# scottjones03/NoisyQuantumSimulator

Hardware: AMD Instinct MI355X
Metric: Lindblad param-points/sec (2-atom Rydberg CZ sweep); achieved HBM GB/s vs peak (higher is better)
Workload: dtype f64; 1 GPU; C2: 10k-point (Omega, Delta) LP-square CZ sweep per GPU, medium apparatus, full reference noise model (8 Lindblad channels); points_per_gpu=10000, global_points=10000, parallelism=range-shard x1, method=chebyshev (auto: 16-lane DPP-row propagator kernel, phase frame)

## Files before the change

noisyquantumsimulator_amd/csrc/ryd_engine.hip:

```cpp
#include <hip/hip_runtime.h>

#include <dlfcn.h>

#include <math.h>
#include <stdint.h>
#include <stdio.h>
#include <string.h>

#include <algorithm>
#include <atomic>
#include <chrono>
#include <complex>
#include <condition_variable>
#include <mutex>
#include <string>
#include <thread>
#include <type_traits>
#include <utility>
#include <vector>

#include "../../include/ryd_engine.h"

struct ryd_slot_work {
  void* dbuf = nullptr;
  size_t dcap = 0;
  void* hbuf = nullptr;
  size_t hcap = 0;
  hipEvent_t ev[4] = {nullptr, nullptr, nullptr, nullptr};
  bool ev_ok = false;
  hipEvent_t mark[2] = {nullptr, nullptr};
};

struct ryd_handle {
  std::vector<int> dev;
  std::vector<hipStream_t> stream;
  std::vector<ryd_slot_work> work;
  std::vector<double> timeline;
  std::mutex mu;
};

namespace {

constexpr int BLOCK = 256;
constexpr double MILLER_SEED = 1e-200;
constexpr int MILLER_MARGIN = 10;
constexpr double X_SKIP = 1e-20;
constexpr double X_CAP = 2.0e6;

struct PointP {
  double Om, Dl, V, d1;
  double gA[4], gB[4];
  double tau, xr, xi, corr, A, wmod, phoff, otau;
  int nseg;
  int64_t i, ld;
  const double* prm;
};

__device__ __forceinline__ double col(const double* p, int f, int64_t ld, int64_t i) {
  return p[(int64_t)f * ld + i];
}

template <int PROTO, typename Get>
__device__ __forceinline__ PointP load_point_with(Get get) {
  PointP q;
  q.prm = nullptr; q.ld = 0; q.i = 0;
  q.Om = get(RYD_P_OMEGA);
  q.Dl = get(RYD_P_DELTA);
  q.V = get(RYD_P_V);
  q.d1 = get(RYD_P_DELTA1);
#pragma unroll
  for (int c = 0; c < 4; ++c) {
    q.gA[c] = get(RYD_P_G1_A + c);
    q.gB[c] = get(RYD_P_G1_B + c);
  }
  q.tau = get(RYD_P_TAU);
  q.xr = q.xi = q.corr = q.A = q.wmod = q.phoff = q.otau = 0.0;
  q.nseg = 0;
  if (PROTO == RYD_PROTO_LP_SQUARE || PROTO == RYD_PROTO_LP_SHAPED) {
    q.xr = get(RYD_P_XI_RE);
    q.xi = get(RYD_P_XI_IM);
    q.corr = (PROTO == RYD_PROTO_LP_SHAPED) ? get(RYD_P_AREA_CORR) : 1.0;
  } else if (PROTO == RYD_PROTO_SMOOTH_JP) {
    q.A = get(RYD_P_A);
    q.wmod = get(RYD_P_OMEGA_MOD);
    q.phoff = get(RYD_P_PHI_OFF);
  } else {
    q.otau = get(RYD_P_OMEGA_TAU);
    q.nseg = (int)get(RYD_P_NSEG);
  }
  return q;
}

// ... 1382 lines not shown
  }
  const bool in_t = (nseg & 1) != 0;
  if (lane_ok) {
    if (in_t) rotate_coord(Rt[pl], Rs[pl], j, cp, sp);
    else rotate_coord(Rs[pl], Rt[pl], j, cp, sp);
  }
  wave_sync();
  if (!in_t && lane_ok) {
#pragma unroll
    for (int k = 0; k < 4; ++k) Rs[pl][k][j] = Rt[pl][k][j];
  }
  wave_sync();
  if (live) {
#pragma unroll
    for (int k = 0; k < 4; ++k) st[(int64_t)j * lds + 4 * i + k] = Rs[pl][k][j];
  }
  if (live && j == 0) {
    uint32_t stat = status[i];
    double pops[4], tr11 = 0.0;
    bool fin = true;
#pragma unroll
    for (int k = 0; k < 4; ++k) pops[k] = Rs[pl][k][5 * (k >> 1) + (k & 1)];
    for (int r = 0; r < NC; ++r)
      for (int k = 0; k < 4; ++k) fin = fin && isfinite(Rs[pl][k][r]);
#pragma unroll
    for (int a = 0; a < 3; ++a)
#pragma unroll
      for (int b = 0; b < 3; ++b) tr11 += Rs[pl][3][5 * a + b];
    if (!fin) stat |= RYD_STATUS_NONFINITE;
    const double nan = __builtin_nan("");
    const double avg = 0.25 * (pops[0] + pops[1] + pops[2] + pops[3]);
#pragma unroll
    for (int k = 0; k < 4; ++k) {
      sm[(int64_t)(RYD_S_POP0 + k) * ldm + i] = pops[k];
      sm[(int64_t)(RYD_S_OV_RE0 + k) * ldm + i] = nan;
      sm[(int64_t)(RYD_S_OV_IM0 + k) * ldm + i] = nan;
    }
    sm[(int64_t)RYD_S_AVG_POP * ldm + i] = avg;
    sm[(int64_t)RYD_S_CTRL_PHASE * ldm + i] = nan;
    sm[(int64_t)RYD_S_PENALTY * ldm + i] = nan;
    sm[(int64_t)RYD_S_AVG_F * ldm + i] = avg;
    sm[(int64_t)RYD_S_TRACE11 * ldm + i] = tr11;
    status[i] = stat;
  }
}

#ifndef RYD_S16_WAVES
#define RYD_S16_WAVES 4
#endif
#ifndef RYD_LP_UNSQUARED
#define RYD_LP_UNSQUARED 2
#endif
#include "ryd_sym16.inc"
#include "ryd_sched_table.inc"
#include "ryd_sched16.inc"
#include "ryd_ket_sched.inc"

constexpr int DP_BLOCK = 64;

__device__ __forceinline__ void lindblad_rhs(const Gen& A, const Gen& B, double vs,
                                             const double (&y)[25], double (&f)[25]) {
#pragma unroll
  for (int e = 0; e < 25; ++e) f[e] = 0.0;
  apply_A(A, y, f);
  apply_B(B, y, f);
  apply_V(vs, y, f);
}

struct DP {
  static constexpr double a[6][5] = {
      {0, 0, 0, 0, 0},
      {1.0 / 5, 0, 0, 0, 0},
      {3.0 / 40, 9.0 / 40, 0, 0, 0},
      {44.0 / 45, -56.0 / 15, 32.0 / 9, 0, 0},
      {19372.0 / 6561, -25360.0 / 2187, 64448.0 / 6561, -212.0 / 729, 0},
      {9017.0 / 3168, -355.0 / 33, 46732.0 / 5247, 49.0 / 176, -5103.0 / 18656}};
  static constexpr double b[6] = {35.0 / 384, 0, 500.0 / 1113, 125.0 / 192, -2187.0 / 6784, 11.0 / 84};
  static constexpr double e[6] = {71.0 / 57600, 0, -71.0 / 16695, 71.0 / 1920, -17253.0 / 339200,
                                  22.0 / 525};
  static constexpr double e7 = -1.0 / 40;
};

using KStore = double[6][25][DP_BLOCK];

template <int J>
__device__ __forceinline__ void dp_stage_input(const double (&y)[25], double hh, const KStore& ks, int lt,
                                               double (&tmp)[25]) {
#pragma unroll
  for (int e = 0; e < 25; ++e) {
    double acc = 0.0;
#pragma unroll
    for (int l = 0; l < J; ++l) acc = fma(DP::a[J][l], ks[l][e][lt], acc);
    tmp[e] = fma(hh, acc, y[e]);
  }
}

template <int PROTO>
__global__ __launch_bounds__(DP_BLOCK) void lindblad_dopri5_kernel(
    const double* __restrict__ prm, int64_t n, int64_t ldp, double* __restrict__ st, int64_t lds,
    double* __restrict__ sm, int64_t ldm, uint32_t* __restrict__ status, int n_steps, int shape,
    double rtol, double atol, int64_t max_steps) {
  __shared__ KStore ks;
  const int lt = threadIdx.x;
  const int64_t gid = (int64_t)blockIdx.x * DP_BLOCK + lt;
  const bool live = gid < 4 * n;
  const int64_t i = live ? (gid >> 2) : (n - 1);
// ... 536 lines not shown
    uint64_t keep = UINT64_MAX;
    (void)hipMemPoolSetAttribute(p, hipMemPoolAttrReleaseThreshold, &keep);
    pools[dev] = p;
  }
  return pools[dev];
}

int launch_jp_split(const ryd_batch_desc* d, const double* dp, int64_t n, int64_t ldp, double* ds,
                    int64_t lds, double* dm, int64_t ldm, uint32_t* dstat, hipStream_t stream) {
  const bool sym = (d->flags & RYD_FLAG_SYMMETRIC_ATOMS) != 0;
  int dev = 0;
  HIPCHK(hipGetDevice(&dev));
  hipMemPool_t pool = jp_pool(dev);
  if (!pool) return fail(RYD_ERR_ALLOC, "jp workspace pool creation failed");
  double* W = nullptr;
  HIPCHK(hipMallocFromPoolAsync((void**)&W, sizeof(double) * NC * NC * (size_t)n, pool, stream));
  const int ns = d->n_steps, sh = d->shape;
  int rc = launch_typed(sym ? jp_rows_kernel<true> : jp_rows_kernel<false>, (n + PPB - 1) / PPB, BLOCK, 0, stream,
                        dp, n, ldp, W, dm, ldm, dstat, ns, sh);
  if (!rc)
    rc = launch_typed(sym ? jp_frame_kernel<3, true> : jp_frame_kernel<4, false>, (n + FPB - 1) / FPB, BLOCK, 0,
                      stream, dp, n, ldp, W, ds, lds, dm, ldm, dstat, ns);
  hipError_t ef = hipFreeAsync(W, stream);
  if (rc) return rc;
  if (ef != hipSuccess) return fail(RYD_ERR_HIP, std::string("jp workspace free: ") + hipGetErrorString(ef));
  return RYD_OK;
}

template <int PROTO>
int launch_sym16(const double* dp, int64_t n, int64_t ldp, double* ds, int64_t lds, double* dm, int64_t ldm,
                 uint32_t* dstat, int ns, int sh, hipStream_t stream) {
  const int st32 = sym16_store32_enabled() && lds >= 0 && ldm >= 0 && lds <= (0x1fffffffLL - 15) / 3 &&
                   ldm <= (0x1fffffffLL - 3) / 15;
  const int bal = PROTO == RYD_PROTO_LP_SQUARE ? sym16_balance_mode() : 0;
  const int wtm = sym16_wt_mode();
  if (wtm == -2) return fail(RYD_ERR_INVALID, "RYD_S16_WT must be 0, 1 or 3");
  if (bal != 0) {
    const int cus = sym16_device_cus();
    S16Plan pl;
    const bool planned = sym16_plan(n, cus, 0, &pl);
    if (bal == 2 && !planned)
      return fail(RYD_ERR_HIP, "RYD_S16_BALANCE=2: the device's compute-unit count is not available");
    if (planned && (bal == 2 || pl.auto_on)) {
      if (const char* eg = getenv("RYD_S16_BALANCE_GPC")) {
        char* end = nullptr;
        const long over = strtol(eg, &end, 10);
        if (end == eg || *end != '\0' || over < 1 || over > S16_BAL_MAXW)
          return fail(RYD_ERR_INVALID, "RYD_S16_BALANCE_GPC must be an integer from 1 to 16");
        sym16_plan(n, cus, (int)over, &pl);
      }
      const char* eh = getenv("RYD_S16_BALANCE_NOHANDOFF");
      static_assert(RYD_P_XI_IM == 14, "the largest LP-square parameter column");
      const bool p32 = sym16_param32_enabled() && ldp <= (0x7fffffffLL / 8 - n) / 14;
      auto fb = p32 ? lindblad_sym16_kernel<RYD_PROTO_LP_SQUARE, 2> : lindblad_sym16_kernel<RYD_PROTO_LP_SQUARE, 1>;
      if (!ds)
        fb = p32 ? lindblad_sym16_nostate_kernel<RYD_PROTO_LP_SQUARE, 2>
                 : lindblad_sym16_nostate_kernel<RYD_PROTO_LP_SQUARE, 1>;
      const int noh = eh && eh[0] == '1', wt = wtm >= 0 ? wtm : S16_WT_AUTO;
      return launch_typed(fb, pl.workgroups, S16_BLOCK * pl.waves, 0, stream, dp, n, ldp, ds, lds, dm, ldm, dstat,
                          ns, pl.gpc, st32, noh, wt);
    }
  }
  if (wtm > 0) return fail(RYD_ERR_UNSUPPORTED, "RYD_S16_WT: write-through stores need the balanced launch form");
  return launch_typed(ds ? lindblad_sym16_kernel<PROTO> : lindblad_sym16_nostate_kernel<PROTO>,
                      (n + S16_PPW - 1) / S16_PPW, S16_BLOCK, 0, stream, dp, n, ldp, ds, lds, dm, ldm, dstat, ns, sh,
                      st32);
}

int launch_kernels(BatchPath path, const ryd_batch_desc* d, const double* dp, int64_t n, int64_t ldp, double* ds,
                   int64_t lds, double* dm, int64_t ldm, uint32_t* dstat, hipStream_t stream) {
  const bool sym = (d->flags & RYD_FLAG_SYMMETRIC_ATOMS) != 0, dim4 = d->dim == 4;
  const int ns = d->n_steps, sh = d->shape;
  auto go = [&](auto kernel, int64_t blocks, unsigned block, auto... more) {
    return launch_typed(kernel, blocks, block, 0, stream, dp, n, ldp, ds, lds, dm, ldm, dstat, ns, sh,
                        more...);
  };
  if (!ds && !has_twin(path)) return fail(RYD_ERR_UNSUPPORTED, "no kernel for this descriptor");
  return with_protocol(d->protocol, [&](auto proto) -> int {
    constexpr int P = decltype(proto)::value;
    constexpr bool FEW = P != RYD_PROTO_LP_SHAPED;
    KernelFn k = nullptr;
    switch (path) {
      case PATH_DOPRI5:
        return go(lindblad_dopri5_kernel<P>, (4 * n + DP_BLOCK - 1) / DP_BLOCK, DP_BLOCK, d->rtol, d->atol,
                  d->max_steps);
      case PATH_DIM4_PROP:
        if constexpr (FEW) return go(lindblad4_prop_kernel<P>, (n + D4_PPB - 1) / D4_PPB, D4_BLOCK);
        break;
      case PATH_SHAPED16:
        if constexpr (!FEW) return go(lindblad_shaped16_kernel<P>, (n + SH_PPW - 1) / SH_PPW, SH_BLOCK);
        break;
      case PATH_SYM16:
        if constexpr (FEW) return launch_sym16<P>(dp, n, ldp, ds, lds, dm, ldm, dstat, ns, sh, stream);
        break;
      case PATH_JP_SPLIT: return launch_jp_split(d, dp, n, ldp, ds, lds, dm, ldm, dstat, stream);
      case PATH_LINDBLAD_PROP:
        k = sym ? lindblad_prop_kernel<P, true> : lindblad_prop_kernel<P, false>;
        return go(k, (n + PPB - 1) / PPB, BLOCK);
      case PATH_LINDBLAD_CHEB:
        k = dim4 ? (sym ? lindblad4_cheb_kernel<P, true> : lindblad4_cheb_kernel<P, false>)
                 : (sym ? lindblad_cheb_kernel<P, true> : lindblad_cheb_kernel<P, false>);
        return go(k, (4 * n + BLOCK - 1) / BLOCK, BLOCK);
      case PATH_KET_BLOCK:
        k = ds ? (dim4 ? ket_block_kernel<P, 4> : ket_block_kernel<P, 3>)
               : (dim4 ? ket_block_nostate_kernel<P, 4> : ket_block_nostate_kernel<P, 3>);
        return go(k, (n + BLOCK - 1) / BLOCK, BLOCK);
      case PATH_KET_CHEB:
        return go(dim4 ? ket_cheb_kernel<P, 4> : ket_cheb_kernel<P, 3>, (4 * n + BLOCK - 1) / BLOCK, BLOCK);
    }
    return fail(RYD_ERR_UNSUPPORTED, "no kernel for this descriptor");
  });
}

// ... 956 lines not shown
                      int64_t ld_diag, void* stream, float* elapsed_ms) {
  return on_slot(
      h, slot, stream, elapsed_ms, [] { return RYD_OK; },
      [&](hipStream_t s) {
        return launch_derive(desc, d_in, ld_in, n, d_params, ld_params, d_warn, d_diag, ld_diag, s);
      });
}

int ryd_derive(ryd_handle* h, const ryd_derive_desc* desc, const double* in, int64_t n_cols, int64_t ld_in,
               int64_t n, double* params, int64_t ld_params, uint32_t* warn, double* diag, int64_t ld_diag) {
  if (!h || h->dev.empty() || !desc) return fail(RYD_ERR_INVALID, "derive: NULL handle/desc");
  if (n < 0 || n_cols < 0 || ld_params < n || (diag && ld_diag < n) || (n_cols > 0 && (!in || ld_in < n)))
    return fail(RYD_ERR_INVALID, "derive: bad sizes");
  for (int f = 0; f < RYD_DV_NFIELD; ++f)
    if (desc->col[f] >= n_cols) return fail(RYD_ERR_INVALID, "derive: a field's column is beyond n_cols");
  if (n == 0) return RYD_OK;
  if (!params || !warn) return fail(RYD_ERR_INVALID, "derive: NULL output");
  const int dev = h->dev[0];
  hipStream_t s = h->stream[0];
  HIPCHK(hipSetDevice(dev));
  auto al = [](size_t x) { return (x + 255) & ~(size_t)255; };
  const size_t bIn = sizeof(double) * (size_t)n_cols * n, bP = sizeof(double) * RYD_NPARAM * (size_t)n,
               bW = sizeof(uint32_t) * (size_t)n, bD = diag ? sizeof(double) * RYD_DV_NDIAG * (size_t)n : 0;
  const size_t oP = al(bIn), oW = oP + al(bP), oD = oW + al(bW), tot = oD + al(bD) + 256;
  char* buf = nullptr;
  HIPCHK(hipStreamSynchronize(s));
  HIPCHK(hipMalloc((void**)&buf, tot));
  hipError_t e = hipSuccess;
  for (int64_t c = 0; c < n_cols && e == hipSuccess; ++c)
    e = hipMemcpyAsync(buf + sizeof(double) * (size_t)c * n, in + c * ld_in, sizeof(double) * n,
                       hipMemcpyHostToDevice, s);
  if (e == hipSuccess) e = hipStreamSynchronize(s);
  int rc = RYD_OK;
  if (e == hipSuccess)
    rc = launch_derive(desc, (const double*)buf, n, n, (double*)(buf + oP), n, (uint32_t*)(buf + oW),
                       diag ? (double*)(buf + oD) : nullptr, n, s);
  if (e == hipSuccess && rc == RYD_OK) e = hipStreamSynchronize(s);
  for (int f = 0; f < RYD_NPARAM && e == hipSuccess && rc == RYD_OK; ++f)
    e = hipMemcpyAsync(params + f * ld_params, buf + oP + sizeof(double) * (size_t)f * n, sizeof(double) * n,
                       hipMemcpyDeviceToHost, s);
  if (e == hipSuccess && rc == RYD_OK) e = hipMemcpyAsync(warn, buf + oW, bW, hipMemcpyDeviceToHost, s);
  for (int k = 0; diag && k < RYD_DV_NDIAG && e == hipSuccess && rc == RYD_OK; ++k)
    e = hipMemcpyAsync(diag + k * ld_diag, buf + oD + sizeof(double) * (size_t)k * n, sizeof(double) * n,
                       hipMemcpyDeviceToHost, s);
  const hipError_t es = hipStreamSynchronize(s);
  const hipError_t ef = hipFree(buf);
  if (rc) return rc;
  if (e != hipSuccess) return fail(RYD_ERR_HIP, std::string("derive: ") + hipGetErrorString(e));
  if (ef != hipSuccess || es != hipSuccess) return fail(RYD_ERR_HIP, "derive: free/sync failed");
  return RYD_OK;
}

}
```

noisyquantumsimulator_amd/csrc/ryd_sym16.inc:

```

constexpr int S16_BLOCK = 64;
constexpr int S16_PPW = 4;

#ifndef RYD_S16_SETPRIO
#define RYD_S16_SETPRIO 1
#endif
__device__ __forceinline__ bool s16_one_round() {
  return RYD_S16_SETPRIO && gridDim.x <= 256u * 4u * (unsigned)RYD_S16_WAVES;
}
#define S16_PRIO(n) do { if (s16_one_round()) __builtin_amdgcn_s_setprio(n); } while (0)
#ifndef RYD_S16_PRIO_SPLIT
#define RYD_S16_PRIO_SPLIT 1
#endif
#ifdef RYD_S16_PROF
#define S16_MARK(k) (s16_ts[k] = (double)__builtin_readcyclecounter())
#define S16_PROF_ARG , double* s16_ts
#define S16_PROF_PASS , s16_ts
#else
#define S16_MARK(k) ((void)0)
#define S16_PROF_ARG
#define S16_PROF_PASS
#endif

#ifndef RYD_XCD_MAP
// ... 26 lines not shown
  const long long x = __builtin_bit_cast(long long, v);
  const long long y = __builtin_amdgcn_update_dpp(0LL, x, 0x150 + K, 0xF, 0xF, false);
  return __builtin_bit_cast(double, y);
}

template <typename F, int... I>
__device__ __forceinline__ void static_for_impl(F&& f, std::integer_sequence<int, I...>) {
  (f(std::integral_constant<int, I>{}), ...);
}
template <int N, typename F>
__device__ __forceinline__ void static_for(F&& f) {
  static_for_impl(f, std::make_integer_sequence<int, N>{});
}

template <int M, bool NOP>
__device__ __forceinline__ void fmac5_bcast(double& a0, double& a1, double& a2, double& a3, double& a4,
                                            double c0, double c1, double c2, double c3, double c4,
                                            double w) {
  if constexpr (NOP) asm volatile("s_nop 1" ::: "memory");
  asm volatile(
      "v_fmac_f64_dpp %0, %5, %10 row_newbcast:%11 row_mask:0xf bank_mask:0xf\n\t"
      "v_fmac_f64_dpp %1, %6, %10 row_newbcast:%11 row_mask:0xf bank_mask:0xf\n\t"
      "v_fmac_f64_dpp %2, %7, %10 row_newbcast:%11 row_mask:0xf bank_mask:0xf\n\t"
      "v_fmac_f64_dpp %3, %8, %10 row_newbcast:%11 row_mask:0xf bank_mask:0xf\n\t"
      "v_fmac_f64_dpp %4, %9, %10 row_newbcast:%11 row_mask:0xf bank_mask:0xf"
      : "+v"(a0), "+v"(a1), "+v"(a2), "+v"(a3), "+v"(a4)
      : "v"(c0), "v"(c1), "v"(c2), "v"(c3), "v"(c4), "v"(w), "i"(M));
}

template <int M0, bool NOP = true>
__device__ __forceinline__ void dot5_bcast(double& acc, double x, double o0, double o1, double o2, double o3,
                                           double o4) {
#define RYD_DOT5_BODY                                                                          \
  "v_fmac_f64_dpp %0, %1, %2 row_newbcast:%7 row_mask:0xf bank_mask:0xf\n\t"                  \
  "v_fmac_f64_dpp %0, %1, %3 row_newbcast:%8 row_mask:0xf bank_mask:0xf\n\t"                  \
  "v_fmac_f64_dpp %0, %1, %4 row_newbcast:%9 row_mask:0xf bank_mask:0xf\n\t"                  \
  "v_fmac_f64_dpp %0, %1, %5 row_newbcast:%10 row_mask:0xf bank_mask:0xf\n\t"                 \
  "v_fmac_f64_dpp %0, %1, %6 row_newbcast:%11 row_mask:0xf bank_mask:0xf"
  if constexpr (NOP) {
    asm volatile("s_nop 1\n\t" RYD_DOT5_BODY
                 : "+v"(acc)
                 : "v"(x), "v"(o0), "v"(o1), "v"(o2), "v"(o3), "v"(o4), "i"(M0), "i"(M0 + 1), "i"(M0 + 2),
                   "i"(M0 + 3), "i"(M0 + 4));
  } else {
    asm volatile(RYD_DOT5_BODY
                 : "+v"(acc)
                 : "v"(x), "v"(o0), "v"(o1), "v"(o2), "v"(o3), "v"(o4), "i"(M0), "i"(M0 + 1), "i"(M0 + 2),
                   "i"(M0 + 3), "i"(M0 + 4));
  }
#undef RYD_DOT5_BODY
}

typedef const __attribute__((address_space(3))) double lds_zero_t;
__device__ __forceinline__ void square_cols16(const double (&col)[NS], double (&acc)[NS], lds_zero_t* zl) {
  asm volatile("" ::: "memory");
#pragma unroll
  for (int k = 0; k < 5; ++k) acc[k] = 0.0;
#pragma unroll
  for (int k = 5; k < NS; ++k) {
    acc[k] = zl[k - 5];
    asm volatile("" ::: "memory");
  }
  static_for<NS>([&](auto M) {
    constexpr int m = decltype(M)::value;
    const double own = col[m];
    if constexpr (m == 0) {
      asm volatile("s_nop 1\n\tv_fmac_f64_dpp %0, %1, %2 row_newbcast:0 row_mask:0xf bank_mask:0xf"
                   : "+v"(acc[0])
                   : "v"(col[0]), "v"(own));
    } else {
      fmac5_bcast<m, m == 1>(acc[0], acc[1], acc[2], acc[3], acc[4], col[0], col[1], col[2], col[3], col[4],
                             own);
    }
    if constexpr (m >= 5) {
      fmac5_bcast<m, false>(acc[5], acc[6], acc[7], acc[8], acc[9], col[5], col[6], col[7], col[8], col[9], own);
      fmac5_bcast<m, false>(acc[10], acc[11], acc[12], acc[13], acc[14], col[10], col[11], col[12], col[13],
                            col[14], own);
    }
  });
}

__device__ __forceinline__ void fast_sincos(double x, double& s, double& c) {
  const bool ok = fabs(x) < 1e15;
  const double k = rint(x * 0.63661977236758134308);
  double r = fma(-k, 1.5707963267948966, x);
  r = fma(-k, 6.123233995736766e-17, r);
  r = fma(-k, -1.4973849048591698e-33, r);
  const double z = r * r;
  const double ps = fma(z, fma(z, fma(z, fma(z, fma(z, 1.58969099521155010221e-10, -2.50507602534068634195e-08),
                                           2.75573137070700676789e-06), -1.98412698298579493134e-04),
                               8.33333333332248946124e-03), -1.66666666666666324348e-01);
  const double sr = fma(z * r, ps, r);
  const double pc = fma(z, fma(z, fma(z, fma(z, fma(z, -1.13596475577881948265e-11, 2.08757232129817482790e-09),
                                           -2.75573143513906633035e-07), 2.48015872894767294178e-05),
                               -1.38888888888741095749e-03), 4.16666666666666019037e-02);
  const double hz = 0.5 * z, w = 1.0 - hz;
  const double cr = w + (((1.0 - w) - hz) + z * z * pc);
  const int n = (int)fma(-4.0, floor(k * 0.25), k);
  const double a = (n & 1) ? cr : sr, b = (n & 1) ? sr : cr;
  const double nan = __builtin_nan("");
  s = ok ? ((n & 2) ? -a : a) : nan;
  c = ok ? (((n + 1) & 2) ? -b : b) : nan;
}

template <int PROTO>
__device__ __forceinline__ void seg_polar(const PointP& q, int s, int n_steps, bool frame_ok, double& a,
                                          double& c, double& sn, double& dl, double& dt, bool& hold) {
  hold = false;
  dl = q.Dl;
  if (PROTO == RYD_PROTO_LP_SQUARE) {
    dt = q.tau;
    if (s == 0) {
      a = q.Om;
      c = 1.0;
      sn = 0.0;
    } else {
      a = q.Om;
      c = q.xr;
      sn = q.xi;
      if (__builtin_amdgcn_ballot_w64(!frame_ok) != 0 && !frame_ok) {
        const double m = sqrt(q.xr * q.xr + q.xi * q.xi);
        a = q.Om * m;
        c = m > 0.0 ? q.xr / m : 1.0;
        sn = m > 0.0 ? q.xi / m : 0.0;
      }
    }
  } else if (PROTO == RYD_PROTO_SMOOTH_JP) {
    a = q.Om;
    dt = q.tau / (double)n_steps;
    segment_phase<PROTO>(q, s, n_steps, c, sn);
  } else {
    const Seg g = segment<PROTO>(q, s, n_steps, RYD_SHAPE_SQUARE);
// ... 358 lines not shown
#else
  const int sq = min(sqf > keep ? sqf - keep : 0, RYD_S16_SQ_CAP);
  rep = sqf > keep ? keep : sqf;
#endif
#ifndef RYD_S16_SQ_CAP
  rep = sqf - sq;
#endif
  const double sc = act ? 2.0 / omega : 0.0;
  Gen A = make_gen(g, q.d1, q.gA, sc);
  double vs = sc * 0.5 * q.V;
  if (!act) {
    A = Gen{};
    vs = 0.0;
  }
  double v[NS];
  const int nuse0 = nuse;
  bool have = false;
  bool producer = false;
  if constexpr (SPLIT) {
    producer = ho.role == S16_BAL_PRODUCER;
    if (ho.role == S16_BAL_CONSUMER && ho.poll) have = s16_wait_flag(&ho.flag[ho.slot], ho.polls);
  }
  if (!SPLIT || !have) {
    cheb_unit16(v, r, y, act && lane_ok,
                [&](const double (&b)[NS], double (&o)[NS]) { apply_Lsym_re(A, vs, b, o); }, nuse, nexec, zl);
    if (!count) nuse = nuse0;
  }
  S16_MARK(2);
  s16_phase_prio<2>(ho);
  const int sfm = wave_max16(sqf);
  nrep = sfm > keep ? keep : sfm;
#ifndef RYD_S16_SQ_CAP
  const int smx = sfm > keep ? sfm - keep : 0;
#else
  const int smx = min(sfm > keep ? sfm - keep : 0, RYD_S16_SQ_CAP);
#endif
  int it0 = 0, it1 = smx;
  if constexpr (SPLIT) {
    const int hs = min((int)RYD_S16_BAL_HSQ, smx);
    const int l = 16 * p + r;
    if (producer) it1 = hs;
    if (have) {
      it0 = hs;
#pragma unroll
      for (int k = 0; k < NS; ++k) v[k] = ho.cols[ho.slot][k][l];
      nuse = ho.cnt[ho.slot][0][l];
      nexec = ho.cnt[ho.slot][1][l];
    }
  }
  {
    for (int it = it0; it < it1; it += 2) {
      double w[NS];
      if (RYD_S16_PRIO_SPLIT && it == ((smx >> 1) & ~1)) s16_phase_prio<1>(ho);
      if (it < sq) square_cols16(v, w, zl);
      if (it + 1 < sq) {
        square_cols16(w, v, zl);
      } else if (it < sq) {
#pragma unroll
        for (int k = 0; k < NS; ++k) v[k] = w[k];
      }
    }
  }
  if constexpr (SPLIT) {
    if (producer) {
      const int l = 16 * p + r;
#pragma unroll
      for (int k = 0; k < NS; ++k) ho.cols[ho.slot][k][l] = v[k];
      ho.cnt[ho.slot][0][l] = nuse;
      ho.cnt[ho.slot][1][l] = nexec;
#ifdef RYD_S16_PROF
      S16_MARK(3);
      ho.cnt[ho.slot][2][l] = (int)(s16_ts[3] - s16_ts[0]);
      ho.cnt[ho.slot][3][l] = (int)__builtin_amdgcn_s_getreg((4) | (0 << 6) | (31 << 11));
#endif
      __hip_atomic_store(&ho.flag[ho.slot], 1, __ATOMIC_RELEASE, __HIP_MEMORY_SCOPE_WORKGROUP);
      return true;
    }
  }
  if (count) nsq += sqf;
  S16_MARK(3);
  s16_phase_prio<1>(ho);
  wave_sync();
  if (lane_ok) {
    static_for<NS>([&](auto N) {
      constexpr int nn = decltype(N)::value;
      double w;
      if constexpr (nn == SEG_M) w = v[sym_index(3, 3)] - v[sym_index(4, 4)];
      else if constexpr (nn == SEG_Q) w = 2.0 * v[sym_index(3, 4)];
      else if constexpr (nn == SEG_P) w = v[sym_index(3, 3)] + v[sym_index(4, 4)];
      else w = v[seg_old(nn)];
      Ut[p][nn][r] = w;
    });
  }
  wave_sync();
  lds_zero_t* const src = lane_ok ? (lds_zero_t*)&Ut[p][r][0] : zl;
  double R[NS];
#pragma unroll
  for (int m = 0; m < NS; ++m) R[m] = src[m];
  static_for<NS>([&](auto N) {
    constexpr int nn = decltype(N)::value;
    if constexpr (nn == SEG_M) u[nn] = 0.5 * (R[sym_index(3, 3)] - R[sym_index(4, 4)]);
    else if constexpr (nn == SEG_Q) u[nn] = 0.5 * R[sym_index(3, 4)];
    else if constexpr (nn == SEG_P) u[nn] = 0.5 * (R[sym_index(3, 3)] + R[sym_index(4, 4)]);
    else u[nn] = R[seg_old(nn)];
  });
  S16_MARK(4);
  s16_phase_prio<0>(ho);
  return false;
}
// ... 103 lines not shown
  PointP q = load_point_with<PROTO>([&](int f) {
    const char* base = reinterpret_cast<const char*>(prm + ((int64_t)f * ldp + i0));
    asm("" : "+s"(base));
    const s16_gchar* gbase = (const s16_gchar*)base;
    return *reinterpret_cast<const s16_gdouble*>(gbase + off);
  });
  q.prm = prm;
  q.ld = ldp;
  q.i = i0 + (int64_t)(po8 >> 3);
  return q;
}

template <int PROTO>
__device__ __forceinline__ PointP load_point16_row(const double* __restrict__ prm, int64_t ldp, int64_t i0,
                                                   unsigned po8, int r) {
  static_assert(PROTO == RYD_PROTO_LP_SQUARE && RYD_P_XI_IM == NS - 1, "LP square: columns 0 .. 14, one per lane");
  const unsigned f = (unsigned)(r < NS ? r : NS - 1);
  const unsigned off = f * (8u * (unsigned)ldp) + po8;
  const char* base = reinterpret_cast<const char*>(prm + i0);
  asm("" : "+s"(base));
  const double x = *reinterpret_cast<const s16_gdouble*>((const s16_gchar*)base + off);
  double c[NS];
  static_for<NS>([&](auto K) { c[decltype(K)::value] = row_bcast<decltype(K)::value>(x); });
  PointP q = load_point_with<PROTO>([&](int k) { return c[k]; });
  q.prm = prm;
  q.ld = ldp;
  q.i = i0 + (int64_t)(po8 >> 3);
  return q;
}

__device__ __forceinline__ void s16_in_hand(PointP& q) {
  asm volatile("" : "+v"(q.Om), "+v"(q.Dl), "+v"(q.V), "+v"(q.d1), "+v"(q.gA[0]), "+v"(q.gA[1]), "+v"(q.gA[2]),
               "+v"(q.gA[3]), "+v"(q.gB[0]), "+v"(q.gB[1]), "+v"(q.gB[2]), "+v"(q.gB[3]), "+v"(q.tau), "+v"(q.xr),
               "+v"(q.xi));
}
template <int PROTO>
__device__ __forceinline__ bool point_valid_flat(const PointP& q) {
  static_assert(PROTO == RYD_PROTO_LP_SQUARE, "point_valid's LP-square predicates");
  const auto fin = [](double x) { return (int)isfinite(x); };
  int ok = (int)(q.Om > 0.0) & fin(q.Om) & fin(q.V) & fin(q.Dl) & fin(q.d1);
#pragma unroll
  for (int c = 0; c < 4; ++c)
    ok &= (int)(q.gA[c] >= 0.0) & (int)(q.gB[c] >= 0.0) & fin(q.gA[c]) & fin(q.gB[c]);
  return (ok & (int)(q.tau > 0.0) & fin(q.tau)) != 0;
}

template <int PROTO>
__global__ __launch_bounds__(S16_BLOCK) __attribute__((amdgpu_waves_per_eu(PROTO == RYD_PROTO_BANGBANG ? 3 : RYD_S16_WAVES, 8))) void
lindblad_sym16_kernel(const double* __restrict__ prm, int64_t n, int64_t ldp, double* __restrict__ st,
                      int64_t lds, double* __restrict__ sm, int64_t ldm, uint32_t* __restrict__ status,
                      int n_steps, int shape, int st32) {
  (void)shape;
  constexpr int BAL = PROTO < 0 ? 1 : 0;
  constexpr int gpc = 0, nohandoff = 0, wt = 0, p32 = 0;
  constexpr bool STATE = true;
#include "ryd_sym16_body.inc"
}

template <int PROTO>
__global__ __launch_bounds__(S16_BLOCK) __attribute__((amdgpu_waves_per_eu(PROTO == RYD_PROTO_BANGBANG ? 3 : RYD_S16_WAVES, 8))) void
lindblad_sym16_nostate_kernel(const double* __restrict__ prm, int64_t n, int64_t ldp, double* __restrict__ st,
                              int64_t lds, double* __restrict__ sm, int64_t ldm, uint32_t* __restrict__ status,
                              int n_steps, int shape, int st32) {
  (void)shape;
  constexpr int BAL = PROTO < 0 ? 1 : 0;
  constexpr int gpc = 0, nohandoff = 0, wt = 0, p32 = 0;
  constexpr bool STATE = false;
#include "ryd_sym16_body.inc"
}

template <int PROTO, int BAL>
__global__ __launch_bounds__(S16_BLOCK * S16_BAL_MAXW) __attribute__((amdgpu_waves_per_eu(RYD_S16_WAVES, 8))) void
lindblad_sym16_kernel(const double* __restrict__ prm, int64_t n, int64_t ldp, double* __restrict__ st,
                      int64_t lds, double* __restrict__ sm, int64_t ldm, uint32_t* __restrict__ status,
                      int n_steps, int gpc, int st32, int nohandoff, int wt) {
  static_assert(PROTO == RYD_PROTO_LP_SQUARE && (BAL == 1 || BAL == 2), "the balanced form is built for LP square");
  constexpr int p32 = BAL == 2;
  constexpr bool STATE = true;
#include "ryd_sym16_body.inc"
}

template <int PROTO, int BAL>
__global__ __launch_bounds__(S16_BLOCK * S16_BAL_MAXW) __attribute__((amdgpu_waves_per_eu(RYD_S16_WAVES, 8))) void
lindblad_sym16_nostate_kernel(const double* __restrict__ prm, int64_t n, int64_t ldp, double* __restrict__ st,
                              int64_t lds, double* __restrict__ sm, int64_t ldm, uint32_t* __restrict__ status,
                              int n_steps, int gpc, int st32, int nohandoff, int wt) {
  static_assert(PROTO == RYD_PROTO_LP_SQUARE && (BAL == 1 || BAL == 2), "the balanced form is built for LP square");
  constexpr int p32 = BAL == 2;
  constexpr bool STATE = false;
#include "ryd_sym16_body.inc"
}

constexpr int S16_WT_STATE = 1, S16_WT_SUMMARY = 2;
constexpr int S16_WT_AUTO = S16_WT_STATE | S16_WT_SUMMARY;
template <bool WT, typename P, typename T>
__device__ __forceinline__ void s16_store(P* ptr, T v) {
  if constexpr (WT) __hip_atomic_store(ptr, v, __ATOMIC_RELAXED, __HIP_MEMORY_SCOPE_AGENT);
  else *ptr = v;
}

template <bool WT>
__device__ __forceinline__ void s16_store_state(const double (&v)[7], double* __restrict__ st, int64_t lds,
                                                int64_t i0, int l, int cc, bool in, bool st32) {
  if (st32) {
    const unsigned lo = 8u * ((unsigned)cc + (unsigned)(l >> 4) * (unsigned)lds);
    if (in) {
#pragma unroll
      for (int j = 0; j < 7; ++j) {
        if (j < 6 || l < 16) {
          char* bj = reinterpret_cast<char*>(st + (4 * i0 + 4 * j * lds));
          asm("" : "+s"(bj));
          s16_store<WT>(reinterpret_cast<s16_gdouble*>((s16_gchar*)bj + lo), v[j]);
        }
      }
    }
  } else {
    double* dst = st + 4 * i0 + cc;
    if (in) {
#pragma unroll
      for (int j = 0; j < 7; ++j) {
        const int row = (l >> 4) + 4 * j;
        if (j < 6 || l < 16) s16_store<WT>(dst + (int64_t)row * lds, v[j]);
      }
    }
  }
}

template <bool WT>
__device__ __forceinline__ void s16_store_summary(double v, double c, uint32_t stat, double* __restrict__ sm,
                                                  int64_t ldm, uint32_t* __restrict__ status, int64_t i0, int64_t i,
                                                  int r, int p, bool st32) {
  if (st32) {
    char* b0 = reinterpret_cast<char*>(sm + i0);
    char* b1 = reinterpret_cast<char*>(sm + (RYD_S_NMV_USEFUL * ldm + i0));
    char* b2 = reinterpret_cast<char*>(status + i0);
    asm("" : "+s"(b0));
    asm("" : "+s"(b1));
    asm("" : "+s"(b2));
    const unsigned lo = 8u * ((unsigned)r * (unsigned)ldm + (unsigned)p);
    s16_store<WT>(reinterpret_cast<s16_gdouble*>((s16_gchar*)b0 + lo), v);
    if (r < 4) s16_store<WT>(reinterpret_cast<s16_gdouble*>((s16_gchar*)b1 + lo), c);
// ... 102 lines not shown
```

noisyquantumsimulator_amd/csrc/ryd_sym16_body.inc:

```
  constexpr int NW = BAL ? S16_BAL_MAXW : 1;
  __shared__ __attribute__((aligned(16))) double UtW[NW][S16_PPW][NS][16];
  static_assert(sizeof(UtW[0]) >= sizeof(double) * S16_PPW * 4 * NC, "output staging must fit in Ut");
#ifdef RYD_S16_PROF
  double s16_ts[16];
  s16_ts[8] = (double)__builtin_amdgcn_s_memrealtime();
  S16_MARK(0);
  s16_ts[10] = s16_ts[11] = 0.0;
  s16_ts[12] = 0.0;
  int bal_polls = 0;
#endif
  __shared__ double ZlW[NW][16];
  const int wv = BAL ? __builtin_amdgcn_readfirstlane((int)(threadIdx.x >> 6)) : 0;
  double (&Ut)[S16_PPW][NS][16] = UtW[wv];
  double (&Zl)[16] = ZlW[wv];
  const int l = BAL ? (int)(threadIdx.x & 63u) : (int)threadIdx.x;
  const int p = l >> 4, r = l & 15;
  if (l < 16) Zl[l] = 0.0;
  __shared__ double Hcols[2][NS][64];
  __shared__ int Hcnt[2][S16_BAL_NCNT][64];
  __shared__ int Hflag[2];
  S16Role role = {S16_BAL_WHOLE, 0};
  int64_t job = 0;
  if constexpr (BAL != 0) {
    role = s16_bal_role(gpc, wv);
    job = s16_bal_job(blockIdx.x, gridDim.x, role.off);
    if (threadIdx.x < 2) Hflag[threadIdx.x] = 0;
    __syncthreads();
    S16_MARK(12);
    if (job >= (n + S16_PPW - 1) / S16_PPW) return;
    if (role.role != S16_BAL_WHOLE) __builtin_amdgcn_s_setprio(3);
  }
  const int64_t b0 = (BAL ? job : xcd_block(blockIdx.x, gridDim.x)) * S16_PPW;
  const int64_t i0 = b0 < n ? b0 : n - 1;
  const int64_t last = n - 1 - i0;
  const unsigned po8 = 8u * (unsigned)min(p, last < S16_PPW - 1 ? (int)last : S16_PPW - 1);
  PointP q0l;
  if constexpr (p32 != 0) {
    q0l = load_point16_row<PROTO>(prm, ldp, i0, po8, r);
  } else {
    q0l = load_point16<PROTO>(prm, ldp, i0, po8);
  }
  S16_MARK(13);
  if constexpr (BAL != 0) s16_in_hand(q0l);
  const PointP q0 = q0l;
#ifdef RYD_S16_PROF
  asm volatile("s_waitcnt vmcnt(0)" ::"v"(q0.Om), "v"(q0.xi) : "memory");
  S16_MARK(14);
#endif
  bool valid;
  if constexpr (BAL != 0) valid = point_valid_flat<PROTO>(q0);
  else valid = point_valid<PROTO>(q0, n_steps);
  const bool frame_ok =
      !(PROTO == RYD_PROTO_LP_SQUARE) || !valid || fabs(q0.xr * q0.xr + q0.xi * q0.xi - 1.0) <= 1e-14;
  S16_MARK(1);
  if constexpr (BAL != 0) {
    if (role.role == S16_BAL_WHOLE) __builtin_amdgcn_s_setprio(3 - RYD_S16_BAL_PRIO_DROP);
  } else {
    S16_PRIO(3);
  }
#ifndef RYD_S16_TAIL_PRIO
#define RYD_S16_TAIL_PRIO 3
#endif
  if (!BAL && RYD_S16_TAIL_PRIO && !s16_one_round() &&
      blockIdx.x + 256u * 4u * (unsigned)RYD_S16_WAVES >= gridDim.x)
    __builtin_amdgcn_s_setprio(RYD_S16_TAIL_PRIO);
  double t = (r == sym_index(1, 1)) ? 1.0 : 0.0;
  double z = (r == 1) ? 1.0 : 0.0;
  double s00 = 1.0;
  double u[NS];
  double cp = 1.0, sp = 0.0;
  int nuse = 0, nexec = 0, nsq = 0;
  bool over_cap = false;
  const int nseg = n_segments<PROTO>(n_steps);
  SegRot rw_out = {};

  if constexpr (PROTO == RYD_PROTO_SMOOTH_JP) {
    double ph_c, ph_s, dt;
    double th_c, th_s, dc, ds;
    {
      const PointP& q = q0;
// ... 214 lines not shown
```

Baseline: 475.9 million points/s.

## Split balanced sym16 kernel into own TU, mask idle lanes in squaring, drop barrier

The balanced LP-square kernels now live in a separate translation unit with a packed config argument and an explicit workgroup count. This should cut kernel-argument size and keep the rest of the engine from affecting their register allocation. In split mode, the upper part of the column-squaring step runs under an exec mask so lanes whose results are unused stay idle. The startup __syncthreads that reset the hand-off flags is replaced by consumer-only relaxed atomic stores. The trade-offs are inline assembly that hard-codes the exec mask layout, and a possible ordering risk if the barrier was doing more than resetting flags.

```diff
diff --git a/noisyquantumsimulator_amd/csrc/ryd_engine.hip b/noisyquantumsimulator_amd/csrc/ryd_engine.hip
--- a/noisyquantumsimulator_amd/csrc/ryd_engine.hip
+++ b/noisyquantumsimulator_amd/csrc/ryd_engine.hip
@@ -38,6 +38,10 @@
   std::vector<double> timeline;
   std::mutex mu;
 };
+
+__attribute__((visibility("hidden"))) hipError_t ryd_s16_bal_launch(
+    int form, bool state, unsigned workgroups, unsigned block, hipStream_t stream, const double* prm, int64_t n,
+    int64_t ldp, int cfg, double* sm, uint32_t* status, int64_t ldm, double* st, int64_t lds, int n_steps);
 
 namespace {
 
@@ -1526,6 +1530,9 @@
 #define RYD_LP_UNSQUARED 2
 #endif
 #include "ryd_sym16.inc"
+#ifdef RYD_S16_BAL_TU
+}
+#else
 #include "ryd_sched_table.inc"
 #include "ryd_sched16.inc"
 #include "ryd_ket_sched.inc"
@@ -2168,13 +2175,11 @@
       const char* eh = getenv("RYD_S16_BALANCE_NOHANDOFF");
       static_assert(RYD_P_XI_IM == 14, "the largest LP-square parameter column");
       const bool p32 = sym16_param32_enabled() && ldp <= (0x7fffffffLL / 8 - n) / 14;
-      auto fb = p32 ? lindblad_sym16_kernel<RYD_PROTO_LP_SQUARE, 2> : lindblad_sym16_kernel<RYD_PROTO_LP_SQUARE, 1>;
-      if (!ds)
-        fb = p32 ? lindblad_sym16_nostate_kernel<RYD_PROTO_LP_SQUARE, 2>
-                 : lindblad_sym16_nostate_kernel<RYD_PROTO_LP_SQUARE, 1>;
       const int noh = eh && eh[0] == '1', wt = wtm >= 0 ? wtm : S16_WT_AUTO;
-      return launch_typed(fb, pl.workgroups, S16_BLOCK * pl.waves, 0, stream, dp, n, ldp, ds, lds, dm, ldm, dstat,
-                          ns, pl.gpc, st32, noh, wt);
+      if (pl.workgroups > 0x7fffffffLL) return fail(RYD_ERR_INVALID, "batch too large for one launch");
+      HIPCHK(ryd_s16_bal_launch(p32 ? 2 : 1, ds != nullptr, (unsigned)pl.workgroups, S16_BLOCK * pl.waves, stream, dp,
+                                n, ldp, s16_bal_cfg(pl.gpc, st32, noh, wt), dm, dstat, ldm, ds, lds, ns));
+      return RYD_OK;
     }
   }
   if (wtm > 0) return fail(RYD_ERR_UNSUPPORTED, "RYD_S16_WT: write-through stores need the balanced launch form");
@@ -3237,3 +3242,4 @@
 }
 
 }
+#endif
diff --git a/noisyquantumsimulator_amd/csrc/ryd_sym16.inc b/noisyquantumsimulator_amd/csrc/ryd_sym16.inc
--- a/noisyquantumsimulator_amd/csrc/ryd_sym16.inc
+++ b/noisyquantumsimulator_amd/csrc/ryd_sym16.inc
@@ -102,6 +102,38 @@
 }
 
 typedef const __attribute__((address_space(3))) double lds_zero_t;
+
+#ifndef RYD_S16_MASK_IDLE
+#define RYD_S16_MASK_IDLE 1
+#endif
+#define S16_SQ_F(k, kc, m, mc) \
+  "v_fmac_f64_dpp %" #k ", %" #kc ", %" #mc " row_newbcast:" #m " row_mask:0xf bank_mask:0xf\n\t"
+#define S16_SQ_G(m, mc)                                                                                    \
+  S16_SQ_F(0, 16, m, mc) S16_SQ_F(1, 17, m, mc) S16_SQ_F(2, 18, m, mc) S16_SQ_F(3, 19, m, mc)              \
+  S16_SQ_F(4, 20, m, mc) S16_SQ_F(5, 21, m, mc) S16_SQ_F(6, 22, m, mc) S16_SQ_F(7, 23, m, mc)              \
+  S16_SQ_F(8, 24, m, mc) S16_SQ_F(9, 25, m, mc) S16_SQ_F(10, 26, m, mc) S16_SQ_F(11, 27, m, mc)            \
+  S16_SQ_F(12, 28, m, mc) S16_SQ_F(13, 29, m, mc) S16_SQ_F(14, 30, m, mc)
+__device__ __forceinline__ void square_upper_masked(const double (&c)[NS], double (&a)[NS]) {
+  static_assert(NS == 15, "operands 0-14: accumulators, 15: the saved exec, 16-30: columns");
+  uint64_t saved;
+  asm volatile(
+      "s_mov_b64 %15, exec\n\t"
+      "s_and_b32 exec_lo, exec_lo, 0x7fe07fe0\n\t"
+      "s_and_b32 exec_hi, exec_hi, 0x7fe07fe0\n\t"
+      "s_nop 1\n\t"
+      S16_SQ_G(5, 21) S16_SQ_G(6, 22) S16_SQ_G(7, 23) S16_SQ_G(8, 24) S16_SQ_G(9, 25)
+      S16_SQ_G(10, 26) S16_SQ_G(11, 27) S16_SQ_G(12, 28) S16_SQ_G(13, 29) S16_SQ_G(14, 30)
+      "s_mov_b64 exec, %15"
+      : "+v"(a[0]), "+v"(a[1]), "+v"(a[2]), "+v"(a[3]), "+v"(a[4]), "+v"(a[5]), "+v"(a[6]), "+v"(a[7]), "+v"(a[8]),
+        "+v"(a[9]), "+v"(a[10]), "+v"(a[11]), "+v"(a[12]), "+v"(a[13]), "+v"(a[14]), "=&s"(saved)
+      : "v"(c[0]), "v"(c[1]), "v"(c[2]), "v"(c[3]), "v"(c[4]), "v"(c[5]), "v"(c[6]), "v"(c[7]), "v"(c[8]), "v"(c[9]),
+        "v"(c[10]), "v"(c[11]), "v"(c[12]), "v"(c[13]), "v"(c[14])
+      : "scc");
+}
+#undef S16_SQ_G
+#undef S16_SQ_F
+
+template <bool MASK = false>
 __device__ __forceinline__ void square_cols16(const double (&col)[NS], double (&acc)[NS], lds_zero_t* zl) {
   asm volatile("" ::: "memory");
 #pragma unroll
@@ -111,7 +143,7 @@
     acc[k] = zl[k - 5];
     asm volatile("" ::: "memory");
   }
-  static_for<NS>([&](auto M) {
+  static_for<MASK ? 5 : NS>([&](auto M) {
     constexpr int m = decltype(M)::value;
     const double own = col[m];
     if constexpr (m == 0) {
@@ -128,6 +160,7 @@
                             col[14], own);
     }
   });
+  if constexpr (MASK) square_upper_masked(col, acc);
 }
 
 __device__ __forceinline__ void fast_sincos(double x, double& s, double& c) {
@@ -592,9 +625,9 @@
     for (int it = it0; it < it1; it += 2) {
       double w[NS];
       if (RYD_S16_PRIO_SPLIT && it == ((smx >> 1) & ~1)) s16_phase_prio<1>(ho);
-      if (it < sq) square_cols16(v, w, zl);
+      if (it < sq) square_cols16<SPLIT && RYD_S16_MASK_IDLE != 0>(v, w, zl);
       if (it + 1 < sq) {
-        square_cols16(w, v, zl);
+        square_cols16<SPLIT && RYD_S16_MASK_IDLE != 0>(w, v, zl);
       } else if (it < sq) {
 #pragma unroll
         for (int k = 0; k < NS; ++k) v[k] = w[k];
@@ -804,7 +837,7 @@
                       int n_steps, int shape, int st32) {
   (void)shape;
   constexpr int BAL = PROTO < 0 ? 1 : 0;
-  constexpr int gpc = 0, nohandoff = 0, wt = 0, p32 = 0;
+  constexpr int gpc = 0, nohandoff = 0, wt = 0, p32 = 0, nwg = 0;
   constexpr bool STATE = true;
 #include "ryd_sym16_body.inc"
 }
@@ -816,29 +849,34 @@
                               int n_steps, int shape, int st32) {
   (void)shape;
   constexpr int BAL = PROTO < 0 ? 1 : 0;
-  constexpr int gpc = 0, nohandoff = 0, wt = 0, p32 = 0;
+  constexpr int gpc = 0, nohandoff = 0, wt = 0, p32 = 0, nwg = 0;
   constexpr bool STATE = false;
 #include "ryd_sym16_body.inc"
 }
 
+__host__ __device__ constexpr int s16_bal_cfg(int gpc, int st32, int nohandoff, int wt) {
+  return gpc | (st32 ? 32 : 0) | (nohandoff ? 64 : 0) | (wt << 7);
+}
+#define RYD_S16_BAL_PARAMS                                                                                   \
+  const double* __restrict__ prm, int64_t n, int64_t ldp, int cfg, int nwg, double* __restrict__ sm,         \
+      uint32_t* __restrict__ status, int64_t ldm, double* __restrict__ st, int64_t lds, int n_steps
+#define RYD_S16_BAL_UNPACK                                                                                   \
+  static_assert(PROTO == RYD_PROTO_LP_SQUARE && (BAL == 1 || BAL == 2), "the balanced form is built for LP square"); \
+  static_assert(S16_BAL_MAXW < 32, "gpc takes cfg's low five bits");                                         \
+  constexpr int p32 = BAL == 2;                                                                              \
+  const int gpc = cfg & 31, st32 = cfg & 32, nohandoff = cfg & 64, wt = cfg >> 7
 template <int PROTO, int BAL>
 __global__ __launch_bounds__(S16_BLOCK * S16_BAL_MAXW) __attribute__((amdgpu_waves_per_eu(RYD_S16_WAVES, 8))) void
-lindblad_sym16_kernel(const double* __restrict__ prm, int64_t n, int64_t ldp, double* __restrict__ st,
-                      int64_t lds, double* __restrict__ sm, int64_t ldm, uint32_t* __restrict__ status,
-                      int n_steps, int gpc, int st32, int nohandoff, int wt) {
-  static_assert(PROTO == RYD_PROTO_LP_SQUARE && (BAL == 1 || BAL == 2), "the balanced form is built for LP square");
-  constexpr int p32 = BAL == 2;
+lindblad_sym16_kernel(RYD_S16_BAL_PARAMS) {
+  RYD_S16_BAL_UNPACK;
   constexpr bool STATE = true;
 #include "ryd_sym16_body.inc"
 }
 
 template <int PROTO, int BAL>
 __global__ __launch_bounds__(S16_BLOCK * S16_BAL_MAXW) __attribute__((amdgpu_waves_per_eu(RYD_S16_WAVES, 8))) void
-lindblad_sym16_nostate_kernel(const double* __restrict__ prm, int64_t n, int64_t ldp, double* __restrict__ st,
-                              int64_t lds, double* __restrict__ sm, int64_t ldm, uint32_t* __restrict__ status,
-                              int n_steps, int gpc, int st32, int nohandoff, int wt) {
-  static_assert(PROTO == RYD_PROTO_LP_SQUARE && (BAL == 1 || BAL == 2), "the balanced form is built for LP square");
-  constexpr int p32 = BAL == 2;
+lindblad_sym16_nostate_kernel(RYD_S16_BAL_PARAMS) {
+  RYD_S16_BAL_UNPACK;
   constexpr bool STATE = false;
 #include "ryd_sym16_body.inc"
 }
diff --git a/noisyquantumsimulator_amd/csrc/ryd_sym16_bal.hip b/noisyquantumsimulator_amd/csrc/ryd_sym16_bal.hip
--- /dev/null
+++ b/noisyquantumsimulator_amd/csrc/ryd_sym16_bal.hip
@@ -0,0 +1,14 @@
+#define RYD_S16_BAL_TU 1
+#include "ryd_engine.hip"
+
+hipError_t ryd_s16_bal_launch(int form, bool state, unsigned workgroups, unsigned block, hipStream_t stream,
+                              const double* prm, int64_t n, int64_t ldp, int cfg, double* sm, uint32_t* status,
+                              int64_t ldm, double* st, int64_t lds, int n_steps) {
+  constexpr int P = RYD_PROTO_LP_SQUARE;
+  void (*k)(RYD_S16_BAL_PARAMS) =
+      state ? (form == 2 ? lindblad_sym16_kernel<P, 2> : lindblad_sym16_kernel<P, 1>)
+            : (form == 2 ? lindblad_sym16_nostate_kernel<P, 2> : lindblad_sym16_nostate_kernel<P, 1>);
+  int nwg = (int)workgroups;
+  void* args[] = {&prm, &n, &ldp, &cfg, &nwg, &sm, &status, &ldm, &st, &lds, &n_steps};
+  return hipLaunchKernel((const void*)k, dim3(workgroups), dim3(block), args, 0, stream);
+}
diff --git a/noisyquantumsimulator_amd/csrc/ryd_sym16_body.inc b/noisyquantumsimulator_amd/csrc/ryd_sym16_body.inc
--- a/noisyquantumsimulator_amd/csrc/ryd_sym16_body.inc
+++ b/noisyquantumsimulator_amd/csrc/ryd_sym16_body.inc
@@ -23,9 +23,9 @@
   int64_t job = 0;
   if constexpr (BAL != 0) {
     role = s16_bal_role(gpc, wv);
-    job = s16_bal_job(blockIdx.x, gridDim.x, role.off);
-    if (threadIdx.x < 2) Hflag[threadIdx.x] = 0;
-    __syncthreads();
+    job = s16_bal_job(blockIdx.x, nwg, role.off);
+    if (role.role == S16_BAL_CONSUMER)
+      __hip_atomic_store(&Hflag[role.off - (gpc & ~3)], 0, __ATOMIC_RELAXED, __HIP_MEMORY_SCOPE_WORKGROUP);
     S16_MARK(12);
     if (job >= (n + S16_PPW - 1) / S16_PPW) return;
     if (role.role != S16_BAL_WHOLE) __builtin_amdgcn_s_setprio(3);
```

New measurement: 487.2 million points/s (median of 6 runs). +2.4%, better.
